# jayleicn/ClipBERT

Hardware: NVIDIA H100
Metric: clips/sec fwd+bwd MSRVTT ret (ResNet50+BERT-base) (higher is better)
Workload: dtype bf16

## Files before the change

clipbert_b200/csrc/common.cuh:

```cuda
#pragma once
#include <cuda.h>
#include <cuda_bf16.h>
#include <cuda_runtime.h>
#include <stdint.h>

#include "drop_cfg.h"

namespace cb {

#ifndef CB_SPIN_LIMIT
#define CB_SPIN_LIMIT (1u << 24)
#endif

__device__ __forceinline__ uint32_t smem_u32(const void* p) {
  return static_cast<uint32_t>(__cvta_generic_to_shared(p));
}

__device__ __forceinline__ void pdl_wait() { asm volatile("griddepcontrol.wait;" ::: "memory"); }
__device__ __forceinline__ void pdl_trigger() { asm volatile("griddepcontrol.launch_dependents;" ::: "memory"); }

__device__ __forceinline__ void mbar_init(uint64_t* bar, uint32_t count) {
  asm volatile("mbarrier.init.shared::cta.b64 [%0], %1;" ::"r"(smem_u32(bar)), "r"(count));
}
__device__ __forceinline__ void fence_mbar_init() {
  asm volatile("fence.mbarrier_init.release.cluster;" ::: "memory");
}
__device__ __forceinline__ void fence_proxy_async_smem() {
  asm volatile("fence.proxy.async.shared::cta;" ::: "memory");
}
__device__ __forceinline__ void mbar_expect_tx(uint64_t* bar, uint32_t bytes) {
  asm volatile("mbarrier.arrive.expect_tx.shared::cta.b64 _, [%0], %1;" ::"r"(smem_u32(bar)),
               "r"(bytes)
               : "memory");
}
__device__ __forceinline__ void mbar_arrive(uint64_t* bar) {
  asm volatile("mbarrier.arrive.shared::cta.b64 _, [%0];" ::"r"(smem_u32(bar)) : "memory");
}
__device__ __forceinline__ void mbar_arrive_if(uint64_t* bar, bool pred) {
  asm volatile("{\n\t.reg .pred p;\n\tsetp.ne.b32 p, %1, 0;\n\t@p mbarrier.arrive.shared::cta.b64 _, [%0];\n\t}" ::"r"(smem_u32(bar)),
               "r"(static_cast<uint32_t>(pred))
               : "memory");
}
__device__ __forceinline__ bool mbar_try_wait(uint64_t* bar, uint32_t parity) {
  uint32_t ok;
  asm volatile(
      "{\n\t.reg .pred p;\n\t"
      "mbarrier.try_wait.parity.shared::cta.b64 p, [%1], %2, %3;\n\t"
      "selp.u32 %0, 1, 0, p;\n\t}"
      : "=r"(ok)
      : "r"(smem_u32(bar)), "r"(parity), "r"(2000u)
      : "memory");
  return ok != 0;
}
__device__ __forceinline__ void mbar_wait(uint64_t* bar, uint32_t parity) {
  uint32_t spins = 0;
  while (!mbar_try_wait(bar, parity)) {
    if (++spins > CB_SPIN_LIMIT) __trap();
  }
}
__device__ __forceinline__ void mbar_wait_unguarded(uint64_t* bar, uint32_t parity) {
  while (!mbar_try_wait(bar, parity)) {
  }
}

__device__ __forceinline__ void tma_prefetch_desc(const CUtensorMap* map) {
  asm volatile("prefetch.tensormap [%0];" ::"l"(map) : "memory");
}
__device__ __forceinline__ void tma_load_2d(void* smem_dst, const CUtensorMap* map, uint64_t* bar,
                                            int c0, int c1) {
  asm volatile(
      "cp.async.bulk.tensor.2d.shared::cluster.global.mbarrier::complete_tx::bytes "
      "[%0], [%1, {%3, %4}], [%2];" ::"r"(smem_u32(smem_dst)),
      "l"(map), "r"(smem_u32(bar)), "r"(c0), "r"(c1)
      : "memory");
}

__device__ __forceinline__ void bulk_load_1d(uint32_t smem_dst, const void* gsrc, uint32_t bytes, uint64_t* bar) {
  asm volatile("cp.async.bulk.shared::cluster.global.mbarrier::complete_tx::bytes [%0], [%1], %2, [%3];" ::"r"(smem_dst), "l"(gsrc),
               "r"(bytes), "r"(smem_u32(bar))
               : "memory");
}

__device__ __forceinline__ void tma_load_2d_s32(uint32_t smem_dst, const CUtensorMap* map, uint64_t* bar, int c0, int c1) {
  asm volatile(
      "cp.async.bulk.tensor.2d.shared::cluster.global.mbarrier::complete_tx::bytes "
      "[%0], [%1, {%3, %4}], [%2];" ::"r"(smem_dst),
      "l"(map), "r"(smem_u32(bar)), "r"(c0), "r"(c1)
      : "memory");
}

__device__ __forceinline__ void tma_load_3d(void* smem_dst, const CUtensorMap* map, uint64_t* bar, int c0, int c1, int c2) {
  asm volatile(
      "cp.async.bulk.tensor.3d.shared::cluster.global.mbarrier::complete_tx::bytes "
      "[%0], [%1, {%3, %4, %5}], [%2];" ::"r"(smem_u32(smem_dst)),
      "l"(map), "r"(smem_u32(bar)), "r"(c0), "r"(c1), "r"(c2)
      : "memory");
}

__device__ __forceinline__ void tma_store_2d(const CUtensorMap* map, const void* smem_src, int c0, int c1) {
  asm volatile("cp.async.bulk.tensor.2d.global.shared::cta.bulk_group [%0, {%2, %3}], [%1];" ::"l"(map),
               "r"(smem_u32(smem_src)), "r"(c0), "r"(c1)
               : "memory");
}
__device__ __forceinline__ void tma_store_2d_s32(const CUtensorMap* map, uint32_t smem_src, int c0, int c1) {
  asm volatile("cp.async.bulk.tensor.2d.global.shared::cta.bulk_group [%0, {%2, %3}], [%1];" ::"l"(map), "r"(smem_src), "r"(c0), "r"(c1)
               : "memory");
}
__device__ __forceinline__ uint4 lds128(uint32_t saddr) {
  uint4 v;
  asm volatile("ld.shared.v4.u32 {%0, %1, %2, %3}, [%4];" : "=r"(v.x), "=r"(v.y), "=r"(v.z), "=r"(v.w) : "r"(saddr));
  return v;
}
__device__ __forceinline__ void sts128(uint32_t saddr, uint4 v) {
  asm volatile("st.shared.v4.u32 [%0], {%1, %2, %3, %4};" ::"r"(saddr), "r"(v.x), "r"(v.y), "r"(v.z), "r"(v.w) : "memory");
}
__device__ __forceinline__ void tma_store_commit() { asm volatile("cp.async.bulk.commit_group;" ::: "memory"); }
template <int N>
__device__ __forceinline__ void tma_store_wait_read() {
  asm volatile("cp.async.bulk.wait_group.read %0;" ::"n"(N) : "memory");
// ... 222 lines not shown
```

clipbert_b200/csrc/gemm.cu:

```cuda
#include "common.cuh"
#include "host_util.h"

namespace cb {

constexpr int BM = 128;
constexpr int BK = 64;
constexpr int CONSUMER_WARPS = 8;
constexpr int GEMM_THREADS = (CONSUMER_WARPS + 1) * 32;
constexpr int PP_THREADS = 3 * 128;
constexpr int PP_PRODUCER_REGS = 40;
constexpr int PP_CONSUMER_REGS = 232;
constexpr int PP_BAR_TURN = 1;
constexpr int MAX_STAGES = 8;
constexpr int SMEM_LIMIT = 232448;
constexpr int STG_PITCH = 36;
constexpr int STG_WARP_FLOATS = 16 * STG_PITCH;
constexpr int EPI_BYTES = CONSUMER_WARPS * STG_WARP_FLOATS * 4;
constexpr int IN_BOX_BYTES = BM * 64 * 2;

struct GemmEpi {
  const float* scale;
  const float* shift;
  const __nv_bfloat16* residual;
  const __nv_bfloat16* aux;
  int aux_mode;
  int act;
  void* out;
  int64_t out_ld;
  int out_fp32;
  __nv_bfloat16* out2;
  int64_t out2_ld;
  int rowmap, H, W;
  uint32_t drop_thresh;
  float drop_inv_keep;
  uint64_t seed;
  const uint64_t* seed_off;
  int mn3d;
  long long* dbg;
};

__device__ __forceinline__ void dbg_stamp(const GemmEpi& epi, int slot) {
  if (epi.dbg) {
    epi.dbg[blockIdx.x * 32 + slot] = clock64();
    if (slot == 0 || slot == 11) {
      unsigned long long ns;
      asm volatile("mov.u64 %0, %%globaltimer;" : "=l"(ns));
      epi.dbg[blockIdx.x * 32 + (slot == 0 ? 12 : 13)] = static_cast<long long>(ns);
    }
  }
}

template <int BN>
struct GemmCfg {
  static constexpr int A_BYTES = BM * BK * 2;
  static constexpr int B_BYTES = BN * BK * 2;
  static constexpr int STAGE_BYTES = A_BYTES + B_BYTES;
  static constexpr int BAR_BYTES = 256;
};

enum { EK_GENERIC = 0, EK_SHIFT_ACT = 1, EK_RELU_MASK = 2, EK_DROP_RES = 3, EK_GELU_STASH = 4, EK_AUX_MUL = 5 };

template <int NC>
__device__ __forceinline__ void add_shift(float (&f)[NC], const float (&shv)[NC]) {
#pragma unroll
  for (int j = 0; j < NC; ++j) f[j] += shv[j];
}
template <int NC>
__device__ __forceinline__ void add_residual(float (&f)[NC], const uint32_t (&res16)[NC / 2]) {
#pragma unroll
  for (int j = 0; j < NC / 2; ++j) {
    const float2 r2 = unpack_bf16x2(res16[j]);
    f[2 * j] += r2.x;
    f[2 * j + 1] += r2.y;
  }
}
template <int NC>
__device__ __forceinline__ void epilogue_shift_act(float (&f)[NC], const float (&shv)[NC], bool has_shift, const uint32_t (&res16)[NC / 2], bool has_res,
                                                   bool relu) {
  if (has_shift) add_shift<NC>(f, shv);
  if (has_res) add_residual<NC>(f, res16);
  if (relu) {
#pragma unroll
    for (int j = 0; j < NC; ++j) f[j] = fmaxf(f[j], 0.0f);
  }
}
template <int NC>
__device__ __forceinline__ void epilogue_relu_mask(float (&f)[NC], const uint32_t (&res16)[NC / 2], bool has_res, const uint32_t (&aux16)[NC / 2]) {
  if (has_res) add_residual<NC>(f, res16);
#pragma unroll
  for (int j = 0; j < NC / 2; ++j) {
    const uint32_t a = aux16[j];
    f[2 * j] = ((a & 0x8000u) == 0u && (a & 0x7fffu) != 0u) ? f[2 * j] : 0.0f;
    f[2 * j + 1] = ((a & 0x80000000u) == 0u && (a & 0x7fff0000u) != 0u) ? f[2 * j + 1] : 0.0f;
  }
}
template <int NC>
__device__ __forceinline__ void epilogue_drop_res(float (&f)[NC], const float (&shv)[NC], bool has_shift, const uint32_t (&res16)[NC / 2], bool has_res,
                                                  uint64_t dseed, uint64_t didx, uint32_t thresh, float inv_keep) {
  if (has_shift) add_shift<NC>(f, shv);
#pragma unroll
  for (int j = 0; j < NC; j += 4) {
    float m[4];
    dropout_mult4(dseed, didx + j, thresh, inv_keep, m);
    f[j] *= m[0]; f[j + 1] *= m[1]; f[j + 2] *= m[2]; f[j + 3] *= m[3];
  }
  if (has_res) add_residual<NC>(f, res16);
}
template <int NC>
__device__ __forceinline__ void epilogue_gelu_stash(float (&f)[NC], const float (&shv)[NC], bool has_shift, uint32_t (&o2_16)[NC / 2]) {
  if (has_shift) add_shift<NC>(f, shv);
#pragma unroll
  for (int j = 0; j < NC / 2; ++j) {
    float y0, g0, y1, g1;
    gelu_erf_and_grad(f[2 * j], y0, g0);
    gelu_erf_and_grad(f[2 * j + 1], y1, g1);
    f[2 * j] = y0;
    f[2 * j + 1] = y1;
    o2_16[j] = pack_bf16x2(g0, g1);
  }
}
template <int NC>
__device__ __forceinline__ void epilogue_aux_mul(float (&f)[NC], const uint32_t (&res16)[NC / 2], bool has_res, const uint32_t (&aux16)[NC / 2]) {
  if (has_res) add_residual<NC>(f, res16);
#pragma unroll
  for (int j = 0; j < NC / 2; ++j) {
    const float2 a2 = unpack_bf16x2(aux16[j]);
    f[2 * j] *= a2.x;
    f[2 * j + 1] *= a2.y;
  }
}
template <int NC, bool GUARD>
__device__ __forceinline__ void epilogue_math(float (&f)[NC], const GemmEpi& epi, const float (&shv)[NC], bool has_shift, uint64_t dseed, int nb, int N,
                                              int64_t orow, const uint32_t (&res16)[NC / 2], bool has_res, const uint32_t (&aux16)[NC / 2], bool has_aux,
// ... 140 lines not shown
    wgmma_wait<1>();
    wgmma_fence_acc(acc);
    if (prev >= 0) {
      __syncwarp();
      if (lane == 0) mbar_arrive(&empty_bar[prev]);
    }
    prev = s;
    if (++s == STAGES) { s = 0; ph ^= 1; }
  }
  wgmma_wait<0>();
  wgmma_fence_acc(acc);
  if (prev >= 0) {
    __syncwarp();
    if (lane == 0) mbar_arrive(&empty_bar[prev]);
  }
}

template <int BN, int TB>
__device__ __forceinline__ void mma_tile_pp(float (&acc)[2][BN / 2], uint32_t smem0, int stage_bytes, int KCH, int STAGES, int n_iters,
                                            int lane, int& s, uint32_t& ph, uint64_t* full_bar, uint64_t* empty_bar, int pass_bar,
                                            bool in_stage) {
  using Cfg = GemmCfg<BN>;
  int prev = -1;
  for (int i = 0; i < n_iters; i += KCH) {
    const int nch = min(KCH, n_iters - i);
    mbar_wait_unguarded(&full_bar[s], ph);
    __syncwarp();
    wgmma_fence();
    wgmma_fence_acc(acc[0]);
    wgmma_fence_acc(acc[1]);
    for (int ch = 0; ch < nch; ++ch) {
      const uint32_t a_addr = smem0 + s * stage_bytes + ch * Cfg::STAGE_BYTES;
      const uint32_t b_addr = a_addr + Cfg::A_BYTES;
#pragma unroll
      for (int k = 0; k < BK / 16; ++k) {
        const uint64_t bd = TB ? gmma_desc(b_addr + k * 2048, BK * 128, 1024) : gmma_desc(b_addr + k * 32, 16, 1024);
        const uint32_t accum = (i > 0 || ch > 0 || k > 0) ? 1u : 0u;
#pragma unroll
        for (int h = 0; h < 2; ++h) wgmma_bf16<BN, 0, TB>(acc[h], gmma_desc(a_addr + h * (64 * 128) + k * 32, 16, 1024), bd, accum);
      }
    }
    wgmma_commit();
    wgmma_wait<1>();
    wgmma_fence_acc(acc[0]);
    wgmma_fence_acc(acc[1]);
    if (prev >= 0) {
      __syncwarp();
      mbar_arrive_if(&empty_bar[prev], lane == 0);
    }
    prev = s;
    if (++s == STAGES) { s = 0; ph ^= 1; }
    if (pass_bar && i + KCH >= n_iters) {
      if (in_stage) mbar_wait_unguarded(&full_bar[s], ph);
      named_bar_arrive(pass_bar, 2 * 128);
    }
  }
  wgmma_wait<0>();
  wgmma_fence_acc(acc[0]);
  wgmma_fence_acc(acc[1]);
  if (prev >= 0) {
    __syncwarp();
    mbar_arrive_if(&empty_bar[prev], lane == 0);
  }
}

template <int BN>
__device__ __forceinline__ void wgrad_epilogue(const float (&acc)[BN / 2], float* obase, int64_t out_ld, const float* scale, int M, int N, int r0,
                                               int n0, int lane) {
  const int r1 = r0 + 8;
  const float rs0 = (r0 < M && scale) ? scale[r0] : 1.0f;
  const float rs1 = (r1 < M && scale) ? scale[r1] : 1.0f;
#pragma unroll
  for (int j = 0; j < BN / 8; ++j) {
    const int n = n0 + j * 8 + 2 * (lane & 3);
    if (n < N) {
      if (r0 < M) red_add_f32x2(obase + static_cast<int64_t>(r0) * out_ld + n, acc[4 * j] * rs0, acc[4 * j + 1] * rs0);
      if (r1 < M) red_add_f32x2(obase + static_cast<int64_t>(r1) * out_ld + n, acc[4 * j + 2] * rs1, acc[4 * j + 3] * rs1);
    }
  }
}

__device__ __forceinline__ uint32_t swz128(uint32_t box, int r, int q) { return box + r * 128 + ((q ^ (r & 7)) << 4); }

template <int BN, int MODE>
__global__ void __launch_bounds__(PP_THREADS, 1)
    gemm_pingpong_kernel(const __grid_constant__ CUtensorMap tmA, const __grid_constant__ CUtensorMap tmB, const __grid_constant__ CUtensorMap tmR,
                         const __grid_constant__ CUtensorMap tmX, int M, int N, int K, int ntaps, int tap_w, int tap_sign, int tiles_m,
                         int tiles_n, int total_tiles, int STAGES, int KCH, int N_IN, GemmEpi epi) {
  static_assert(MODE != 1 && BN <= 128, "TN / NN tiles of 128 x 64 or 128 x 128");
  using Cfg = GemmCfg<BN>;
  extern __shared__ uint8_t smem_raw[];
  uint8_t* smem = reinterpret_cast<uint8_t*>((reinterpret_cast<uintptr_t>(smem_raw) + 1023) & ~static_cast<uintptr_t>(1023));
  const int stage_bytes = KCH * Cfg::STAGE_BYTES;
  const bool has_res = epi.residual != nullptr, has_aux = epi.aux != nullptr;
  constexpr int IN_TILE_BYTES = (BN / 64) * IN_BOX_BYTES;
  const int in_bytes = (has_res + has_aux) * IN_TILE_BYTES;
  uint8_t* in_base = smem + STAGES * stage_bytes;
  uint8_t* stg_base = in_base + N_IN * in_bytes;
  uint64_t* full_bar = reinterpret_cast<uint64_t*>(stg_base + EPI_BYTES);
  uint64_t* empty_bar = full_bar + MAX_STAGES;
  uint64_t* in_full = empty_bar + MAX_STAGES;
  uint64_t* in_empty = in_full + 2;

  const int warp = __shfl_sync(0xffffffffu, static_cast<int>(threadIdx.x >> 5), 0);
  const int lane = threadIdx.x & 31;
  const int unit = blockIdx.x;
  const int n_units = gridDim.x;
  if (threadIdx.x == 0) dbg_stamp(epi, 0);
  pdl_trigger();
  if (threadIdx.x == 0) {
    tma_prefetch_desc(&tmA);
    tma_prefetch_desc(&tmB);
    if (has_res) tma_prefetch_desc(&tmR);
    if (has_aux) tma_prefetch_desc(&tmX);
    for (int s = 0; s < STAGES; ++s) {
      mbar_init(&full_bar[s], 1);
      mbar_init(&empty_bar[s], 4);
    }
    for (int b = 0; b < 2; ++b) {
      mbar_init(&in_full[b], 1);
      mbar_init(&in_empty[b], 4);
    }
    fence_mbar_init();
  }
  __syncthreads();
  const int kc_per_tap = (K + BK - 1) / BK;
  const int n_iters = ntaps * kc_per_tap;
  const bool in_stage = in_bytes && !N_IN;
  const int tile_stages = (n_iters + KCH - 1) / KCH + (in_stage ? 1 : 0);
  pdl_wait();
  if (threadIdx.x == 0) dbg_stamp(epi, 1);

  if (warp < 4) {
    setmaxnreg_dec<PP_PRODUCER_REGS>();
    if (warp == 0 && lane == 0) {
      constexpr int B_BOXES = (MODE == 0) ? 1 : BN / 64;
      int s = 0;
      uint32_t ph = 0;
      auto load_inputs = [&](int tile) {
        const TileInfo t = decode_tile<BN, MODE>(tile, tiles_m, tiles_n, K, ntaps, 0);
        uint64_t* bar;
        uint8_t* dst;
        if (N_IN) {
          const int local = (tile - unit) / n_units;
          const int b = N_IN == 2 ? (local & 1) : 0;
          const int uses = N_IN == 2 ? (local >> 1) : local;
          mbar_wait(&in_empty[b], (static_cast<uint32_t>(uses) & 1u) ^ 1u);
          bar = &in_full[local & 1];
          dst = in_base + b * in_bytes;
        } else {
          mbar_wait(&empty_bar[s], ph ^ 1);
          bar = &full_bar[s];
          dst = smem + s * stage_bytes;
          if (++s == STAGES) { s = 0; ph ^= 1; }
        }
        mbar_expect_tx(bar, in_bytes);
        if (has_res) {
#pragma unroll
          for (int j = 0; j < BN / 64; ++j) tma_load_2d(dst + j * IN_BOX_BYTES, &tmR, bar, t.n0 + j * 64, t.m0);
          dst += IN_TILE_BYTES;
        }
        if (has_aux) {
#pragma unroll
          for (int j = 0; j < BN / 64; ++j) tma_load_2d(dst + j * IN_BOX_BYTES, &tmX, bar, t.n0 + j * 64, t.m0);
        }
      };
      int pend = -1;
      for (int tile = unit; tile < total_tiles; tile += n_units) {
        const TileInfo t = decode_tile<BN, MODE>(tile, tiles_m, tiles_n, K, ntaps, 0);
        const bool inputs_first = tile < unit + N_IN * n_units;
        if (in_bytes && N_IN && inputs_first) load_inputs(tile);
        for (int i = 0; i < n_iters; i += KCH) {
          const int nch = min(KCH, n_iters - i);
          mbar_wait(&empty_bar[s], ph ^ 1);
          mbar_expect_tx(&full_bar[s], nch * Cfg::STAGE_BYTES);
          int tp = 0, kc = i;
          if (ntaps > 1) { tp = i / kc_per_tap; kc = i - tp * kc_per_tap; }
          for (int ch = 0; ch < nch; ++ch) {
            uint8_t* sa = smem + s * stage_bytes + ch * Cfg::STAGE_BYTES;
            uint8_t* sb = sa + Cfg::A_BYTES;
            int shift = 0;
            if (ntaps == 9) shift = tap_sign * ((tp / 3 - 1) * tap_w + (tp % 3 - 1));
            else if (ntaps > 1) shift = tap_sign * tp * tap_w;
            tma_load_2d(sa, &tmA, &full_bar[s], kc * BK, t.m0 + shift);
            if (MODE == 0) {
              tma_load_2d(sb, &tmB, &full_bar[s], tp * K + kc * BK, t.nb0);
            } else if (epi.mn3d) {
              tma_load_3d(sb, &tmB, &full_bar[s], 0, kc * BK, (tp * N + t.nb0) >> 6);
            } else {
#pragma unroll
              for (int j = 0; j < B_BOXES; ++j) tma_load_2d(sb + j * (BK * 128), &tmB, &full_bar[s], tp * N + t.nb0 + j * 64, kc * BK);
            }
            if (++kc == kc_per_tap) { kc = 0; ++tp; }
          }
          if (++s == STAGES) { s = 0; ph ^= 1; }
          if (i == 0 && tile == unit) dbg_stamp(epi, 2);
        }
        if (in_stage) load_inputs(tile);
        if (pend >= 0) load_inputs(pend);
        pend = (in_bytes && N_IN && !inputs_first) ? tile : -1;
      }
      if (pend >= 0) load_inputs(pend);
      dbg_stamp(epi, 3);
    }
    return;
  }

  setmaxnreg_inc<PP_CONSUMER_REGS>();
  const int wg = (warp >> 2) - 1;
  const int wq = warp & 3;
  const uint32_t smem0 = smem_u32(smem);
  const uint64_t dseed = epi.drop_thresh ? drop_seed(epi.seed, epi.seed_off) : 0ull;
  float acc[2][BN / 2];
  int s = 0;
  uint32_t ph = 0;
  auto ring_skip = [&](int n) {
    s += n;
    while (s >= STAGES) { s -= STAGES; ph ^= 1; }
  };
  if (wg == 1) ring_skip(tile_stages);

  const int er = lane & 15, eh = lane >> 4;
  float* stg = reinterpret_cast<float*>(stg_base) + (warp - 4) * STG_WARP_FLOATS;
  const bool has_out2 = epi.out2 != nullptr;
  const bool has_shift = epi.shift != nullptr;
  const bool full = (N & 15) == 0 && epi.scale == nullptr;
  const bool drop = epi.drop_thresh != 0;
  int kind = EK_GENERIC;
  if (full) {
    if (!drop && !has_out2 && !has_aux && (epi.act == CB_ACT_NONE || epi.act == CB_ACT_RELU)) kind = EK_SHIFT_ACT;
    else if (!drop && !has_out2 && !has_shift && has_aux && epi.aux_mode == CB_AUX_RELU_MASK && epi.act == CB_ACT_NONE) kind = EK_RELU_MASK;
    else if (drop && !has_out2 && !has_aux && epi.act == CB_ACT_NONE) kind = EK_DROP_RES;
    else if (!drop && has_out2 && !has_aux && !has_res && epi.act == CB_ACT_GELU_STASH_GRAD) kind = EK_GELU_STASH;
    else if (!drop && !has_out2 && !has_shift && has_aux && epi.aux_mode == CB_AUX_MUL && epi.act == CB_ACT_NONE) kind = EK_AUX_MUL;
  }
  const bool kind_relu = epi.act == CB_ACT_RELU;
  const bool guard = (N & 15) != 0;

  for (int local = wg, tile = unit + wg * n_units; tile < total_tiles; local += 2, tile += 2 * n_units) {
    const TileInfo t = decode_tile<BN, MODE>(tile, tiles_m, tiles_n, K, ntaps, 0);
    if (local > 0) named_bar_sync(PP_BAR_TURN + wg, 2 * 128);
    const int pass = tile + n_units < total_tiles ? PP_BAR_TURN + (wg ^ 1) : 0;
    mma_tile_pp<BN, MODE != 0>(acc, smem0, stage_bytes, KCH, STAGES, n_iters, lane, s, ph, full_bar, empty_bar, pass, in_stage);

    const uint32_t in_buf = N_IN ? smem_u32(in_base) + (N_IN == 2 ? wg : 0) * in_bytes : smem0 + s * stage_bytes;
    if (in_bytes) {
      if (N_IN) mbar_wait_unguarded(&in_full[wg], static_cast<uint32_t>(local >> 1) & 1u);
      else mbar_wait_unguarded(&full_bar[s], ph);
    }
    int orow_half[2];
#pragma unroll
    for (int h = 0; h < 2; ++h) {
      const int m = t.m0 + h * 64 + wq * 16 + er;
      bool row_ok = m < M;
      int64_t orow = m;
      if (epi.rowmap == CB_ROWMAP_PAD) {
        const int hw = epi.H * epi.W;
        const int img = m / hw;
        const int r = m - img * hw;
        const int y = r / epi.W, x = r - y * epi.W;
        orow = (static_cast<int64_t>(img) * (epi.H + 2) + y + 1) * (epi.W + 2) + x + 1;
      } else if (epi.rowmap == CB_ROWMAP_UNPAD) {
        const int wp = epi.W + 2, hp = epi.H + 2;
        const int img = m / (hp * wp);
        const int r = m - img * (hp * wp);
        const int y = r / wp, x = r - y * wp;
        row_ok = row_ok && y >= 1 && y <= epi.H && x >= 1 && x <= epi.W;
        orow = (static_cast<int64_t>(img) * epi.H + (y - 1)) * epi.W + (x - 1);
      }
      orow_half[h] = row_ok ? static_cast<int>(orow) : -1;
    }
#pragma unroll
    for (int sc = 0; sc < BN / 32; ++sc) {
#pragma unroll 1
      for (int h = 0; h < 2; ++h) {
        const int wrow = h * 64 + wq * 16;
        __syncwarp();
#pragma unroll
        for (int jj = 0; jj < 4; ++jj) {
          const int j = sc * 4 + jj;
          float* p = stg + (lane >> 2) * STG_PITCH + jj * 8 + 2 * (lane & 3);
          const bool h1 = h != 0;
          *reinterpret_cast<float2*>(p) = make_float2(h1 ? acc[1][4 * j] : acc[0][4 * j], h1 ? acc[1][4 * j + 1] : acc[0][4 * j + 1]);
          *reinterpret_cast<float2*>(p + 8 * STG_PITCH) =
              make_float2(h1 ? acc[1][4 * j + 2] : acc[0][4 * j + 2], h1 ? acc[1][4 * j + 3] : acc[0][4 * j + 3]);
        }
        __syncwarp();
        const int nb = t.n0 + sc * 32 + eh * 16;
        const int64_t orow = h ? orow_half[1] : orow_half[0];
        if (orow < 0 || nb >= N) continue;
        constexpr int NC = 16;
        float f[NC];
        const uint32_t srow = smem_u32(stg + er * STG_PITCH + eh * 16);
#pragma unroll
        for (int j = 0; j < NC / 4; ++j) {
          const uint4 u = lds128(srow + j * 16);
          f[4 * j] = __uint_as_float(u.x); f[4 * j + 1] = __uint_as_float(u.y);
          f[4 * j + 2] = __uint_as_float(u.z); f[4 * j + 3] = __uint_as_float(u.w);
        }
        uint32_t res16[NC / 2], aux16[NC / 2];
        const int tc = sc * 32 + eh * 16;
        const int q = (tc & 63) >> 3;
        if (has_res) {
#pragma unroll
          for (int j = 0; j < 2; ++j) {
            const uint4 u = lds128(swz128(in_buf + (tc >> 6) * IN_BOX_BYTES, wrow + er, q + j));
            res16[4 * j] = u.x; res16[4 * j + 1] = u.y; res16[4 * j + 2] = u.z; res16[4 * j + 3] = u.w;
          }
        }
        if (has_aux) {
#pragma unroll
          for (int j = 0; j < 2; ++j) {
            const uint4 u = lds128(swz128(in_buf + (has_res ? IN_TILE_BYTES : 0) + (tc >> 6) * IN_BOX_BYTES, wrow + er, q + j));
            aux16[4 * j] = u.x; aux16[4 * j + 1] = u.y; aux16[4 * j + 2] = u.z; aux16[4 * j + 3] = u.w;
          }
        }
        float shv[NC];
        if (has_shift) {
#pragma unroll
          for (int j = 0; j < NC; j += 4) {
            float4 s4 = make_float4(0.f, 0.f, 0.f, 0.f);
            if (nb + j + 4 <= N) s4 = __ldg(reinterpret_cast<const float4*>(epi.shift + nb + j));
            shv[j] = s4.x; shv[j + 1] = s4.y; shv[j + 2] = s4.z; shv[j + 3] = s4.w;
          }
        }
        uint32_t o2_16[NC / 2];
        switch (kind) {
          case EK_SHIFT_ACT: epilogue_shift_act<NC>(f, shv, has_shift, res16, has_res, kind_relu); break;
          case EK_RELU_MASK: epilogue_relu_mask<NC>(f, res16, has_res, aux16); break;
          case EK_DROP_RES:
            epilogue_drop_res<NC>(f, shv, has_shift, res16, has_res, dseed, static_cast<uint64_t>(orow) * static_cast<uint64_t>(N) + nb,
                                  epi.drop_thresh, epi.drop_inv_keep);
            break;
          case EK_GELU_STASH: epilogue_gelu_stash<NC>(f, shv, has_shift, o2_16); break;
          case EK_AUX_MUL: epilogue_aux_mul<NC>(f, res16, has_res, aux16); break;
          default:
            if (guard) epilogue_math<NC, true>(f, epi, shv, has_shift, dseed, nb, N, orow, res16, has_res, aux16, has_aux, o2_16, has_out2);
            else epilogue_math<NC, false>(f, epi, shv, has_shift, dseed, nb, N, orow, res16, has_res, aux16, has_aux, o2_16, has_out2);
        }
        if (epi.out_fp32) {
          float* o = reinterpret_cast<float*>(epi.out) + orow * epi.out_ld + nb;
#pragma unroll
          for (int j = 0; j < NC; j += 4)
            if (nb + j + 4 <= N) *reinterpret_cast<float4*>(o + j) = make_float4(f[j], f[j + 1], f[j + 2], f[j + 3]);
        } else {
          __nv_bfloat16* o = reinterpret_cast<__nv_bfloat16*>(epi.out) + orow * epi.out_ld + nb;
#pragma unroll
          for (int j = 0; j < 2; ++j)
            if (nb + 8 * j + 8 <= N)
              *reinterpret_cast<uint4*>(o + 8 * j) = make_uint4(pack_bf16x2(f[8 * j], f[8 * j + 1]), pack_bf16x2(f[8 * j + 2], f[8 * j + 3]),
                                                                pack_bf16x2(f[8 * j + 4], f[8 * j + 5]), pack_bf16x2(f[8 * j + 6], f[8 * j + 7]));
        }
        if (has_out2) {
          __nv_bfloat16* o = epi.out2 + orow * epi.out2_ld + nb;
#pragma unroll
          for (int j = 0; j < 2; ++j)
            if (nb + 8 * j + 8 <= N) *reinterpret_cast<uint4*>(o + 8 * j) = make_uint4(o2_16[4 * j], o2_16[4 * j + 1], o2_16[4 * j + 2], o2_16[4 * j + 3]);
        }
      }
    }
    if (in_bytes) {
      __syncwarp();
      if (lane == 0) mbar_arrive(N_IN ? &in_empty[N_IN == 2 ? wg : 0] : &empty_bar[s]);
      if (!N_IN && ++s == STAGES) { s = 0; ph ^= 1; }
    }
    ring_skip(tile_stages);
  }
  if (threadIdx.x == 4 * 32) dbg_stamp(epi, 11);
}

template <int BN>
__global__ void __launch_bounds__(GEMM_THREADS, 1)
    gemm_kernel(const __grid_constant__ CUtensorMap tmA, const __grid_constant__ CUtensorMap tmB, int M, int N, int K, int ntaps, int tap_w,
                int tap_sign, int iters_per_split, int tiles_m, int tiles_n, int total_tiles, int STAGES, int KCH, GemmEpi epi) {
  using Cfg = GemmCfg<BN>;
  extern __shared__ uint8_t smem_raw[];
  uint8_t* smem = reinterpret_cast<uint8_t*>((reinterpret_cast<uintptr_t>(smem_raw) + 1023) & ~static_cast<uintptr_t>(1023));
  const int stage_bytes = KCH * Cfg::STAGE_BYTES;
  uint64_t* full_bar = reinterpret_cast<uint64_t*>(smem + STAGES * stage_bytes);
  uint64_t* empty_bar = full_bar + MAX_STAGES;

  const int warp = __shfl_sync(0xffffffffu, static_cast<int>(threadIdx.x >> 5), 0);
  const int lane = threadIdx.x & 31;
  const int unit = blockIdx.x;
  const int n_units = gridDim.x;
  if (threadIdx.x == 0) dbg_stamp(epi, 0);
  pdl_trigger();
  if (threadIdx.x == 0) {
    tma_prefetch_desc(&tmA);
    tma_prefetch_desc(&tmB);
    for (int s = 0; s < STAGES; ++s) {
      mbar_init(&full_bar[s], 1);
      mbar_init(&empty_bar[s], CONSUMER_WARPS);
    }
    fence_mbar_init();
  }
  __syncthreads();
  pdl_wait();
  if (threadIdx.x == 0) dbg_stamp(epi, 1);

  if (warp >= CONSUMER_WARPS) {
    if (warp == CONSUMER_WARPS && lane == 0) {
      int s = 0;
      uint32_t ph = 0;
      for (int tile = unit; tile < total_tiles; tile += n_units) {
        const TileInfo t = decode_tile<BN, 1>(tile, tiles_m, tiles_n, K, ntaps, iters_per_split);
        int shift = 0;
        if (ntaps == 9) shift = tap_sign * ((t.tap / 3 - 1) * tap_w + (t.tap % 3 - 1));
        for (int i = 0; i < t.n_iters; i += KCH) {
          const int nch = min(KCH, t.n_iters - i);
          mbar_wait(&empty_bar[s], ph ^ 1);
          mbar_expect_tx(&full_bar[s], nch * Cfg::STAGE_BYTES);
          int kit = t.it_begin + i;
          for (int ch = 0; ch < nch; ++ch, ++kit) {
            uint8_t* sa = smem + s * stage_bytes + ch * Cfg::STAGE_BYTES;
            uint8_t* sb = sa + Cfg::A_BYTES;
            const int p = kit * BK;
            if (epi.mn3d) {
              tma_load_3d(sa, &tmA, &full_bar[s], 0, p, t.m0 >> 6);
              tma_load_3d(sb, &tmB, &full_bar[s], 0, p + shift, t.nb0 >> 6);
            } else {
#pragma unroll
              for (int j = 0; j < BM / 64; ++j) tma_load_2d(sa + j * (BK * 128), &tmA, &full_bar[s], t.m0 + j * 64, p);
#pragma unroll
              for (int j = 0; j < BN / 64; ++j) tma_load_2d(sb + j * (BK * 128), &tmB, &full_bar[s], t.nb0 + j * 64, p + shift);
            }
          }
          if (++s == STAGES) { s = 0; ph ^= 1; }
          if (i == 0 && tile == unit) dbg_stamp(epi, 2);
        }
      }
      dbg_stamp(epi, 3);
    }
    return;
  }

  const int wg = warp >> 2;
  const int wrow = wg * 64 + (warp & 3) * 16;
  const uint32_t smem0 = smem_u32(smem);
  float acc[BN / 2];
  int s = 0;
  uint32_t ph = 0;
  int local = 0;
  for (int tile = unit; tile < total_tiles; tile += n_units, ++local) {
    const TileInfo t = decode_tile<BN, 1>(tile, tiles_m, tiles_n, K, ntaps, iters_per_split);
    if (local == 0 && warp == 0 && lane == 0) dbg_stamp(epi, 4);
    mma_tile<BN, 1, 1>(acc, smem0, stage_bytes, KCH, STAGES, t.n_iters, wg, lane, s, ph, full_bar, empty_bar);
    if (local == 0 && warp == 0 && lane == 0) dbg_stamp(epi, 5);
    wgrad_epilogue<BN>(acc, reinterpret_cast<float*>(epi.out) + static_cast<int64_t>(t.tap) * N, epi.out_ld, epi.scale, M, N,
                       t.m0 + wrow + (lane >> 2), t.n0, lane);
    if (local == 0 && warp == 0 && lane == 0) dbg_stamp(epi, 8);
  }
  if (threadIdx.x == 0) dbg_stamp(epi, 11);
}

static int g_sm_limit = 0;
static int sm_count() {
  static int n = 0;
  if (n == 0) {
    int dev = 0;
    cudaGetDevice(&dev);
    cudaDeviceGetAttribute(&n, cudaDevAttrMultiProcessorCount, dev);
    if (n <= 0) n = 132;
  }
  return (g_sm_limit > 0 && g_sm_limit < n) ? g_sm_limit : n;
}

static long long* g_gemm_timeline = nullptr;
static int g_force_kch = 0;
static int g_mn3d = 1;


struct SmemPlan {
  int epi_bytes, kch, stages, chunk_bytes, n_in;
};
static SmemPlan plan_ring(int bn, bool staging, int kiters, int force_kch, int in_bytes, int n_in) {
  SmemPlan p;
  const int limit = SMEM_LIMIT;
  p.chunk_bytes = BM * BK * 2 + bn * BK * 2;
  p.epi_bytes = staging ? EPI_BYTES : 0;
  p.n_in = n_in;
  const int chunks_fit = (limit - 1024 - GemmCfg<64>::BAR_BYTES - p.epi_bytes - n_in * in_bytes) / p.chunk_bytes;
  const int min_stages = kiters > chunks_fit ? 3 : 2;
  p.kch = 1;
  if (force_kch > 0) p.kch = force_kch;
  else if (g_force_kch > 0) p.kch = g_force_kch;
  else if (kiters >= 4 && chunks_fit >= 4 * min_stages) p.kch = 4;
  else if (kiters >= 2 && chunks_fit >= 2 * min_stages) p.kch = 2;
  if (p.kch > kiters) p.kch = kiters;
  if (p.kch > 1 && chunks_fit / p.kch < 2) p.kch = 1;
  p.stages = chunks_fit / p.kch;
  if (p.stages > MAX_STAGES) p.stages = MAX_STAGES;
  const int stage_iters = ceil_div(kiters, p.kch);
  const int cap = staging ? 2 * stage_iters + 1 : (stage_iters + 1 > 2 ? stage_iters + 1 : 2);
  if (p.stages > cap) p.stages = cap;
  return p;
}
static SmemPlan plan_smem(int bn, bool staging, int kiters, int force_kch = 0, int in_bytes = 0) {
  const SmemPlan none = plan_ring(bn, staging, kiters, force_kch, 0, 0);
  if (in_bytes == 0) return none;
  const SmemPlan two = plan_ring(bn, staging, kiters, force_kch, in_bytes, 2);
  if (two.stages >= 2 && two.stages * two.kch >= kiters) return two;
  if (kiters > 4 && none.stages >= 2 && none.kch * none.chunk_bytes >= in_bytes) return none;
  return plan_ring(bn, staging, kiters, force_kch, in_bytes, 1);
}
static int epi_in_bytes(const cb_gemm_desc& d, int bn) {
  return d.mode == CB_GEMM_WGRAD ? 0 : ((d.residual != nullptr) + (d.aux != nullptr)) * (bn / 64) * IN_BOX_BYTES;
}

template <int BN, int MODE>
static int launch_gemm(const cb_gemm_desc& d, const GemmEpi& epi_in, cudaStream_t stream) {
  static_assert(MODE == 1 || BN <= 128, "TN / NN: 128 x 64 or 128 x 128 tiles");
  GemmEpi epi = epi_in;
  using Cfg = GemmCfg<BN>;
  static bool attr_set = false;
  auto kern = [] {
    if constexpr (MODE == 1) return gemm_kernel<BN>;
    else return gemm_pingpong_kernel<BN, MODE>;
  }();
  if (!attr_set) {
    cudaError_t e = cudaFuncSetAttribute(kern, cudaFuncAttributeMaxDynamicSharedMemorySize, SMEM_LIMIT);
    if (e != cudaSuccess) {
      set_error("cudaFuncSetAttribute(smem=%d): %s", SMEM_LIMIT, cudaGetErrorString(e));
      return CB_ERR_CUDA;
    }
    attr_set = true;
  }
  alignas(64) CUtensorMap ta, tb, tr, tx;
  bool mn3d = false;
  int iters_per_split = 0;
  const int tiles_m = ceil_div(d.m, BM), tiles_n = ceil_div(d.n, BN);
  int total = tiles_m * tiles_n;
  int kiters;
  bool ok;
  if (MODE == 0) {
    ok = get_tmap_2d(&ta, d.a, d.k, d.a_rows, d.a_ld, BK, BM) &&
         get_tmap_2d(&tb, d.b, static_cast<uint64_t>(d.k) * d.ntaps, d.b_rows, d.b_ld, BK, BN);
    kiters = ceil_div(d.k, BK) * d.ntaps;
  } else if (MODE == 2) {
    ok = get_tmap_2d(&ta, d.a, d.k, d.a_rows, d.a_ld, BK, BM);
    mn3d = g_mn3d && d.n % 64 == 0 &&
           get_tmap_3d_mn(&tb, d.b, static_cast<uint64_t>(d.n) * d.ntaps, d.b_rows, d.b_ld, BK, BN / 64);
    if (!mn3d) ok = ok && get_tmap_2d(&tb, d.b, static_cast<uint64_t>(d.n) * d.ntaps, d.b_rows, d.b_ld, 64, BK);
    kiters = ceil_div(d.k, BK) * d.ntaps;
  } else {
    mn3d = g_mn3d && d.m % 64 == 0 && d.n % 64 == 0 && get_tmap_3d_mn(&ta, d.a, d.m, d.a_rows, d.a_ld, BK, BM / 64) &&
           get_tmap_3d_mn(&tb, d.b, d.n, d.b_rows, d.b_ld, BK, BN / 64);
    ok = mn3d || (get_tmap_2d(&ta, d.a, d.m, d.a_rows, d.a_ld, 64, BK) && get_tmap_2d(&tb, d.b, d.n, d.b_rows, d.b_ld, 64, BK));
    const int kc = ceil_div(d.k, BK);
    int splits = d.split_k < 1 ? 1 : d.split_k;
    if (splits > kc) splits = kc;
    iters_per_split = ceil_div(kc, splits);
    splits = ceil_div(kc, iters_per_split);
    total *= splits * d.ntaps;
    kiters = iters_per_split;
  }
  tr = ta;
  tx = ta;
  if (MODE != 1 && d.residual) ok = ok && get_tmap_2d(&tr, d.residual, d.n, d.m, d.res_ld, 64, BM);
  if (MODE != 1 && d.aux) ok = ok && get_tmap_2d(&tx, d.aux, d.n, d.m, d.aux_ld, 64, BM);
  if (!ok) return CB_ERR_CUDA;
  epi.mn3d = mn3d ? 1 : 0;
  const int units = sm_count();
  const int grid = total < units ? total : units;
  const int in_bytes = epi_in_bytes(d, BN);
  const SmemPlan sp = plan_smem(BN, MODE != 1, kiters, (d.reserved >> 8) & 15, in_bytes);
  const int kch = sp.kch, stages = sp.stages;
  if (stages < 2) {
    set_error("cb_gemm: not enough shared memory for a 2-stage pipeline (BN=%d, epilogue %d B + inputs %d B)", BN, sp.epi_bytes,
              in_bytes);
    return CB_ERR_INVALID;
  }
  const int smem_bytes = stages * kch * Cfg::STAGE_BYTES + sp.n_in * in_bytes + sp.epi_bytes + Cfg::BAR_BYTES + 1024;
  if constexpr (MODE == 1)
    launch_gemm_k(kern, grid, GEMM_THREADS, smem_bytes, stream, ta, tb, d.m, d.n, d.k, d.ntaps, d.tap_w, d.tap_sign, iters_per_split,
                  tiles_m, tiles_n, total, stages, kch, epi);
  else
    launch_gemm_k(kern, grid, PP_THREADS, smem_bytes, stream, ta, tb, tr, tx, d.m, d.n, d.k, d.ntaps, d.tap_w, d.tap_sign, tiles_m,
                  tiles_n, total, stages, kch, sp.n_in, epi);
  return check_launch("cb_gemm");
}

struct LaunchCfg {
  int bn, splits;
};

static LaunchCfg choose_config(const cb_gemm_desc& d) {
  const int units = sm_count();
  const int kc = ceil_div(d.k, BK);
  const bool wgrad = d.mode == CB_GEMM_WGRAD;
  const int block_n = (!wgrad && d.block_n == 256) ? 128 : d.block_n;
  static const int cand[3] = {64, 128, 256};
  LaunchCfg best = {64, 1};
  double best_cost = 1e30;
  for (int c = 0; c < 3; ++c) {
    const int bn = cand[c];
    if (block_n && bn != block_n) continue;
    if (!wgrad && bn == 256) continue;
    if (bn > 64 && d.n <= bn / 2) continue;
    const int64_t base = static_cast<int64_t>(ceil_div(d.m, BM)) * ceil_div(d.n, bn) * (wgrad ? d.ntaps : 1);
    const int max_split = wgrad ? (d.split_k > 0 ? d.split_k : (kc < 32 ? kc : 32)) : 1;
    for (int sp = (wgrad && d.split_k > 0) ? d.split_k : 1; sp <= max_split; ++sp) {
      const int ips = ceil_div(wgrad ? kc : kc * d.ntaps, sp);
      const int real_sp = wgrad ? ceil_div(kc, ips) : 1;
      const int64_t tiles = base * real_sp;
      const double rounds = static_cast<double>((tiles + units - 1) / units);
      const SmemPlan pl = plan_smem(bn, !wgrad, ips, (d.reserved >> 8) & 15, epi_in_bytes(d, bn));
      if (pl.stages < 2) continue;
      const double shallow = (pl.stages * pl.kch < 3 && ips > 2) ? 3.0 : 1.0;
      const double stage_cost = 450.0 + pl.kch * pl.chunk_bytes / 60.0;
      const double main_loop = ceil_div(ips, pl.kch) * stage_cost * shallow;
      double cost;
      if (wgrad) {
        cost = rounds * (main_loop + bn * 24.0) + 2500.0;
      } else {
        const double epi = bn * 30.0;
        const double per_tile = main_loop > 0.5 * (main_loop + epi) ? main_loop : 0.5 * (main_loop + epi);
        cost = rounds * per_tile + 0.5 * epi + 2500.0;
      }
      if (cost < best_cost) {
        best_cost = cost;
        best = {bn, real_sp};
      }
    }
  }
  return best;
}

constexpr int WG_MAX_PROBLEMS = 8;
struct WgradProblem {
  CUtensorMap tmA, tmB;
  float* out;
  const float* scale;
  int64_t out_ld;
  int M, N, K;
  int ntaps, tap_w, tap_sign;
  int iters_per_split, tiles_m, tiles_n;
  int tile_begin;
  int mn3d;
};
struct WgradGroup {
  int nprob, total_tiles;
  WgradProblem p[WG_MAX_PROBLEMS];
};
struct WgTile {
  int pi, m0, n0, tap, it_begin, n_iters;
};
__device__ __forceinline__ WgTile wg_decode(const WgradGroup& g, int tile) {
  WgTile t;
  int pi = 0;
  while (pi + 1 < g.nprob && tile >= g.p[pi + 1].tile_begin) ++pi;
  const WgradProblem& P = g.p[pi];
  int r = tile - P.tile_begin;
  const int nt = r % P.tiles_n;
  r /= P.tiles_n;
  const int mt = r % P.tiles_m;
  r /= P.tiles_m;
  t.pi = pi;
  t.m0 = mt * BM;
  t.tap = r % P.ntaps;
  const int split = r / P.ntaps;
  const int kc = (P.K + BK - 1) / BK;
// ... 266 lines not shown
```

Before: 3973.

## Write pingpong GEMM epilogue outputs through swizzled smem and TMA stores

Adds a TMA_OUT variant of the pingpong GEMM kernel. The epilogue packs bf16 results into a swizzled shared-memory tile, and one thread then issues TMA 2D stores for the output and optional second output, replacing per-thread global stores. The launcher enables it only for bf16, non-rowmapped, aligned outputs, and only when the extra double-buffered output smem keeps the pipeline ring depth or the K loop is short. It also adds debug cycle counters. The cost is less smem for stages, an extra named barrier, and a wait for the TMA store to finish reading smem before reuse.

```diff
diff --git a/clipbert_b200/csrc/common.cuh b/clipbert_b200/csrc/common.cuh
--- a/clipbert_b200/csrc/common.cuh
+++ b/clipbert_b200/csrc/common.cuh
@@ -35,6 +35,9 @@
 }
 __device__ __forceinline__ void mbar_arrive(uint64_t* bar) {
   asm volatile("mbarrier.arrive.shared::cta.b64 _, [%0];" ::"r"(smem_u32(bar)) : "memory");
+}
+__device__ __forceinline__ void mbar_arrive_cnt(uint64_t* bar, uint32_t count) {
+  asm volatile("mbarrier.arrive.shared::cta.b64 _, [%0], %1;" ::"r"(smem_u32(bar)), "r"(count) : "memory");
 }
 __device__ __forceinline__ void mbar_arrive_if(uint64_t* bar, bool pred) {
   asm volatile("{\n\t.reg .pred p;\n\tsetp.ne.b32 p, %1, 0;\n\t@p mbarrier.arrive.shared::cta.b64 _, [%0];\n\t}" ::"r"(smem_u32(bar)),
diff --git a/clipbert_b200/csrc/gemm.cu b/clipbert_b200/csrc/gemm.cu
--- a/clipbert_b200/csrc/gemm.cu
+++ b/clipbert_b200/csrc/gemm.cu
@@ -11,6 +11,7 @@
 constexpr int PP_PRODUCER_REGS = 40;
 constexpr int PP_CONSUMER_REGS = 232;
 constexpr int PP_BAR_TURN = 1;
+constexpr int PP_BAR_EPI = 3;
 constexpr int MAX_STAGES = 8;
 constexpr int SMEM_LIMIT = 232448;
 constexpr int STG_PITCH = 36;
@@ -49,6 +50,10 @@
     }
   }
 }
+__device__ __forceinline__ void dbg_accum(const GemmEpi& epi, int slot, bool start) {
+  const long long c = clock64();
+  atomicAdd(reinterpret_cast<unsigned long long*>(epi.dbg + blockIdx.x * 32 + slot), static_cast<unsigned long long>(start ? -c : c));
+}
 
 template <int BN>
 struct GemmCfg {
@@ -355,10 +360,11 @@
 
 __device__ __forceinline__ uint32_t swz128(uint32_t box, int r, int q) { return box + r * 128 + ((q ^ (r & 7)) << 4); }
 
-template <int BN, int MODE>
+template <int BN, int MODE, bool TMA_OUT>
 __global__ void __launch_bounds__(PP_THREADS, 1)
     gemm_pingpong_kernel(const __grid_constant__ CUtensorMap tmA, const __grid_constant__ CUtensorMap tmB, const __grid_constant__ CUtensorMap tmR,
-                         const __grid_constant__ CUtensorMap tmX, int M, int N, int K, int ntaps, int tap_w, int tap_sign, int tiles_m,
+                         const __grid_constant__ CUtensorMap tmX, const __grid_constant__ CUtensorMap tmO,
+                         const __grid_constant__ CUtensorMap tmO2, int M, int N, int K, int ntaps, int tap_w, int tap_sign, int tiles_m,
                          int tiles_n, int total_tiles, int STAGES, int KCH, int N_IN, GemmEpi epi) {
   static_assert(MODE != 1 && BN <= 128, "TN / NN tiles of 128 x 64 or 128 x 128");
   using Cfg = GemmCfg<BN>;
@@ -369,7 +375,9 @@
   constexpr int IN_TILE_BYTES = (BN / 64) * IN_BOX_BYTES;
   const int in_bytes = (has_res + has_aux) * IN_TILE_BYTES;
   uint8_t* in_base = smem + STAGES * stage_bytes;
-  uint8_t* stg_base = in_base + N_IN * in_bytes;
+  const int out_bytes = (TMA_OUT && !in_bytes) ? (1 + (epi.out2 != nullptr)) * IN_TILE_BYTES : 0;
+  uint8_t* out_base = in_base + N_IN * in_bytes;
+  uint8_t* stg_base = out_base + 2 * out_bytes;
   uint64_t* full_bar = reinterpret_cast<uint64_t*>(stg_base + EPI_BYTES);
   uint64_t* empty_bar = full_bar + MAX_STAGES;
   uint64_t* in_full = empty_bar + MAX_STAGES;
@@ -386,6 +394,8 @@
     tma_prefetch_desc(&tmB);
     if (has_res) tma_prefetch_desc(&tmR);
     if (has_aux) tma_prefetch_desc(&tmX);
+    if (TMA_OUT) tma_prefetch_desc(&tmO);
+    if (TMA_OUT && epi.out2) tma_prefetch_desc(&tmO2);
     for (int s = 0; s < STAGES; ++s) {
       mbar_init(&full_bar[s], 1);
       mbar_init(&empty_bar[s], 4);
@@ -513,10 +523,17 @@
   for (int local = wg, tile = unit + wg * n_units; tile < total_tiles; local += 2, tile += 2 * n_units) {
     const TileInfo t = decode_tile<BN, MODE>(tile, tiles_m, tiles_n, K, ntaps, 0);
     if (local > 0) named_bar_sync(PP_BAR_TURN + wg, 2 * 128);
+    if (epi.dbg && wq == 0 && lane == 0) dbg_accum(epi, 16 + wg, true);
     const int pass = tile + n_units < total_tiles ? PP_BAR_TURN + (wg ^ 1) : 0;
     mma_tile_pp<BN, MODE != 0>(acc, smem0, stage_bytes, KCH, STAGES, n_iters, lane, s, ph, full_bar, empty_bar, pass, in_stage);
-
-    const uint32_t in_buf = N_IN ? smem_u32(in_base) + (N_IN == 2 ? wg : 0) * in_bytes : smem0 + s * stage_bytes;
+    if (epi.dbg && wq == 0 && lane == 0) {
+      dbg_accum(epi, 16 + wg, false);
+      dbg_accum(epi, 14 + wg, true);
+    }
+
+    const uint32_t in_buf = !in_bytes ? smem_u32(out_base) + wg * out_bytes
+                                      : N_IN ? smem_u32(in_base) + (N_IN == 2 ? wg : 0) * in_bytes : smem0 + s * stage_bytes;
+    const uint32_t out_buf = in_buf;
     if (in_bytes) {
       if (N_IN) mbar_wait_unguarded(&in_full[wg], static_cast<uint32_t>(local >> 1) & 1u);
       else mbar_wait_unguarded(&full_bar[s], ph);
@@ -611,6 +628,20 @@
             if (guard) epilogue_math<NC, true>(f, epi, shv, has_shift, dseed, nb, N, orow, res16, has_res, aux16, has_aux, o2_16, has_out2);
             else epilogue_math<NC, false>(f, epi, shv, has_shift, dseed, nb, N, orow, res16, has_res, aux16, has_aux, o2_16, has_out2);
         }
+        if constexpr (TMA_OUT) {
+#pragma unroll
+          for (int j = 0; j < 2; ++j)
+            sts128(swz128(out_buf + (tc >> 6) * IN_BOX_BYTES, wrow + er, q + j),
+                   make_uint4(pack_bf16x2(f[8 * j], f[8 * j + 1]), pack_bf16x2(f[8 * j + 2], f[8 * j + 3]),
+                              pack_bf16x2(f[8 * j + 4], f[8 * j + 5]), pack_bf16x2(f[8 * j + 6], f[8 * j + 7])));
+          if (has_out2) {
+#pragma unroll
+            for (int j = 0; j < 2; ++j)
+              sts128(swz128(out_buf + IN_TILE_BYTES + (tc >> 6) * IN_BOX_BYTES, wrow + er, q + j),
+                     make_uint4(o2_16[4 * j], o2_16[4 * j + 1], o2_16[4 * j + 2], o2_16[4 * j + 3]));
+          }
+          continue;
+        }
         if (epi.out_fp32) {
           float* o = reinterpret_cast<float*>(epi.out) + orow * epi.out_ld + nb;
 #pragma unroll
@@ -632,10 +663,30 @@
         }
       }
     }
-    if (in_bytes) {
-      __syncwarp();
-      if (lane == 0) mbar_arrive(N_IN ? &in_empty[N_IN == 2 ? wg : 0] : &empty_bar[s]);
-      if (!N_IN && ++s == STAGES) { s = 0; ph ^= 1; }
+    uint64_t* in_free = N_IN ? &in_empty[N_IN == 2 ? wg : 0] : &empty_bar[s];
+    if constexpr (TMA_OUT) {
+      fence_proxy_async_smem();
+      named_bar_sync(PP_BAR_EPI + wg, 128);
+      if (wq == 0 && lane == 0) {
+#pragma unroll
+        for (int j = 0; j < BN / 64; ++j) tma_store_2d_s32(&tmO, out_buf + j * IN_BOX_BYTES, t.n0 + j * 64, t.m0);
+        if (has_out2) {
+#pragma unroll
+          for (int j = 0; j < BN / 64; ++j) tma_store_2d_s32(&tmO2, out_buf + IN_TILE_BYTES + j * IN_BOX_BYTES, t.n0 + j * 64, t.m0);
+        }
+        tma_store_commit();
+        if (epi.dbg) dbg_accum(epi, 14 + wg, false);
+        tma_store_wait_read<0>();
+        if (in_bytes) mbar_arrive_cnt(in_free, 4);
+      }
+      if (in_bytes && !N_IN && ++s == STAGES) { s = 0; ph ^= 1; }
+    } else {
+      if (epi.dbg && wq == 0 && lane == 0) dbg_accum(epi, 14 + wg, false);
+      if (in_bytes) {
+        __syncwarp();
+        if (lane == 0) mbar_arrive(in_free);
+        if (!N_IN && ++s == STAGES) { s = 0; ph ^= 1; }
+      }
     }
     ring_skip(tile_stages);
   }
@@ -747,13 +798,13 @@
 struct SmemPlan {
   int epi_bytes, kch, stages, chunk_bytes, n_in;
 };
-static SmemPlan plan_ring(int bn, bool staging, int kiters, int force_kch, int in_bytes, int n_in) {
+static SmemPlan plan_ring(int bn, bool staging, int kiters, int force_kch, int in_bytes, int n_in, int out_bytes = 0) {
   SmemPlan p;
   const int limit = SMEM_LIMIT;
   p.chunk_bytes = BM * BK * 2 + bn * BK * 2;
   p.epi_bytes = staging ? EPI_BYTES : 0;
   p.n_in = n_in;
-  const int chunks_fit = (limit - 1024 - GemmCfg<64>::BAR_BYTES - p.epi_bytes - n_in * in_bytes) / p.chunk_bytes;
+  const int chunks_fit = (limit - 1024 - GemmCfg<64>::BAR_BYTES - p.epi_bytes - n_in * in_bytes - out_bytes) / p.chunk_bytes;
   const int min_stages = kiters > chunks_fit ? 3 : 2;
   p.kch = 1;
   if (force_kch > 0) p.kch = force_kch;
@@ -781,24 +832,23 @@
   return d.mode == CB_GEMM_WGRAD ? 0 : ((d.residual != nullptr) + (d.aux != nullptr)) * (bn / 64) * IN_BOX_BYTES;
 }
 
+template <typename Kern>
+static bool smem_opt_in(Kern kern, bool& done) {
+  if (done) return true;
+  cudaError_t e = cudaFuncSetAttribute(kern, cudaFuncAttributeMaxDynamicSharedMemorySize, SMEM_LIMIT);
+  if (e != cudaSuccess) {
+    set_error("cudaFuncSetAttribute(smem=%d): %s", SMEM_LIMIT, cudaGetErrorString(e));
+    return false;
+  }
+  done = true;
+  return true;
+}
+
 template <int BN, int MODE>
 static int launch_gemm(const cb_gemm_desc& d, const GemmEpi& epi_in, cudaStream_t stream) {
   static_assert(MODE == 1 || BN <= 128, "TN / NN: 128 x 64 or 128 x 128 tiles");
   GemmEpi epi = epi_in;
   using Cfg = GemmCfg<BN>;
-  static bool attr_set = false;
-  auto kern = [] {
-    if constexpr (MODE == 1) return gemm_kernel<BN>;
-    else return gemm_pingpong_kernel<BN, MODE>;
-  }();
-  if (!attr_set) {
-    cudaError_t e = cudaFuncSetAttribute(kern, cudaFuncAttributeMaxDynamicSharedMemorySize, SMEM_LIMIT);
-    if (e != cudaSuccess) {
-      set_error("cudaFuncSetAttribute(smem=%d): %s", SMEM_LIMIT, cudaGetErrorString(e));
-      return CB_ERR_CUDA;
-    }
-    attr_set = true;
-  }
   alignas(64) CUtensorMap ta, tb, tr, tx;
   bool mn3d = false;
   int iters_per_split = 0;
@@ -838,19 +888,41 @@
   const int grid = total < units ? total : units;
   const int in_bytes = epi_in_bytes(d, BN);
   const SmemPlan sp = plan_smem(BN, MODE != 1, kiters, (d.reserved >> 8) & 15, in_bytes);
-  const int kch = sp.kch, stages = sp.stages;
+  int kch = sp.kch, stages = sp.stages;
   if (stages < 2) {
     set_error("cb_gemm: not enough shared memory for a 2-stage pipeline (BN=%d, epilogue %d B + inputs %d B)", BN, sp.epi_bytes,
               in_bytes);
     return CB_ERR_INVALID;
   }
-  const int smem_bytes = stages * kch * Cfg::STAGE_BYTES + sp.n_in * in_bytes + sp.epi_bytes + Cfg::BAR_BYTES + 1024;
-  if constexpr (MODE == 1)
-    launch_gemm_k(kern, grid, GEMM_THREADS, smem_bytes, stream, ta, tb, d.m, d.n, d.k, d.ntaps, d.tap_w, d.tap_sign, iters_per_split,
-                  tiles_m, tiles_n, total, stages, kch, epi);
-  else
-    launch_gemm_k(kern, grid, PP_THREADS, smem_bytes, stream, ta, tb, tr, tx, d.m, d.n, d.k, d.ntaps, d.tap_w, d.tap_sign, tiles_m,
-                  tiles_n, total, stages, kch, sp.n_in, epi);
+  alignas(64) CUtensorMap to = ta, to2 = ta;
+  bool tma_out = MODE != 1 && d.rowmap == CB_ROWMAP_NONE && !d.out_fp32 && (reinterpret_cast<uintptr_t>(d.out) & 15) == 0 &&
+                 (!d.out2 || (!in_bytes && (reinterpret_cast<uintptr_t>(d.out2) & 15) == 0)) && !((d.reserved >> 12) & 1);
+  int out_bytes = 0;
+  if (tma_out && !in_bytes) {
+    out_bytes = 2 * (1 + (d.out2 != nullptr)) * (BN / 64) * IN_BOX_BYTES;
+    const SmemPlan po = plan_ring(BN, true, kiters, (d.reserved >> 8) & 15, 0, 0, out_bytes);
+    const bool keeps_ring = po.stages == stages && po.kch == kch;
+    const bool short_loop = kiters <= 12 && po.stages >= 2 && po.stages * po.kch >= 4;
+    if (keeps_ring || short_loop) stages = po.stages, kch = po.kch;
+    else tma_out = false, out_bytes = 0;
+  }
+  if (tma_out) {
+    ok = get_tmap_2d(&to, d.out, d.n, d.m, d.out_ld, 64, BM) && (!d.out2 || get_tmap_2d(&to2, d.out2, d.n, d.m, d.out2_ld, 64, BM));
+    if (!ok) return CB_ERR_CUDA;
+  }
+  const int smem_bytes = stages * kch * Cfg::STAGE_BYTES + sp.n_in * in_bytes + out_bytes + sp.epi_bytes + Cfg::BAR_BYTES + 1024;
+  if constexpr (MODE == 1) {
+    static bool attr_set = false;
+    if (!smem_opt_in(gemm_kernel<BN>, attr_set)) return CB_ERR_CUDA;
+    launch_gemm_k(gemm_kernel<BN>, grid, GEMM_THREADS, smem_bytes, stream, ta, tb, d.m, d.n, d.k, d.ntaps, d.tap_w, d.tap_sign,
+                  iters_per_split, tiles_m, tiles_n, total, stages, kch, epi);
+  } else {
+    static bool attr_set[2] = {false, false};
+    auto kern = tma_out ? gemm_pingpong_kernel<BN, MODE, true> : gemm_pingpong_kernel<BN, MODE, false>;
+    if (!smem_opt_in(kern, attr_set[tma_out])) return CB_ERR_CUDA;
+    launch_gemm_k(kern, grid, PP_THREADS, smem_bytes, stream, ta, tb, tr, tx, to, to2, d.m, d.n, d.k, d.ntaps, d.tap_w, d.tap_sign,
+                  tiles_m, tiles_n, total, stages, kch, sp.n_in, epi);
+  }
   return check_launch("cb_gemm");
 }
 
```

After: 4032 (median of 6 runs). 1.01x the previous value.
